# N3b3x/openballbot-rl

Measured on AMD Instinct MI355X. Metric: env-steps/sec at 4096 envs per GPU (flat terrain, random actions), higher is better.
Workload: dtype f64

## Files before the change

### openballbot-rl_amd/ballbot_gym/_native.py

```python
from __future__ import annotations

import ctypes as C
import os
from pathlib import Path

PKG = Path(__file__).resolve().parent
LIB_PATH = PKG / "_lib" / "libbb_mi355x.so"
SERIAL_LIB_PATH = PKG / "_lib" / "libbb_mi355x_serial.so"
SERIAL_FLAGS = ["-DBB_NO_TWIN_KIN", "-DBB_NO_TWIN_POS", "-DBB_NO_TWIN_BIAS", "-DBB_NO_MODEL_ONCE",
                "-DBB_NO_PRE_BATCH", "-DBB_NO_PRISM_WINDOW"]
CSRC = PKG.parent / "csrc"
INCLUDE = PKG.parent.parent / "include"

NQ, NV, NOBS, HF_N = 17, 15, 15, 293
DONE_TERMINATED, DONE_FAILURE, DONE_DIVERGED, DONE_OVERFLOW = 1, 2, 4, 8
NSTATS = 8
REWARD_DIRECTIONAL, REWARD_DISTANCE, REWARD_NONE = 0, 1, 2
DSBL_PASSIVE, DSBL_GRAVITY = 32, 64


class NativeLibraryError(RuntimeError):
    pass


class BBParams(C.Structure):
    _fields_ = [
        ("max_ep_steps", C.c_int),
        ("max_allowed_tilt", C.c_float),
        ("max_wheel_velocity", C.c_float),
        ("reward_scale", C.c_float),
        ("action_reg_coef", C.c_float),
        ("survival_bonus", C.c_float),
        ("target_dir", C.c_float * 2),
        ("reward_kind", C.c_int),
        ("goal", C.c_float * 2),
        ("goal_scale", C.c_float),
        ("n_terrains", C.c_int),
        ("seed", C.c_uint64),
        ("fp64", C.c_int),
        ("solver_maxiter", C.c_int),
        ("solver_tol", C.c_double),
        ("opt_timestep", C.c_double),
        ("opt_disableflags", C.c_int),
    ]


class PerlinCfg(C.Structure):
    _fields_ = [
        ("scale", C.c_double),
        ("octaves", C.c_int),
        ("persistence", C.c_float),
        ("lacunarity", C.c_float),
        ("amplitude", C.c_double),
    ]


class PPOMlpArgs(C.Structure):
    _fields_ = [(name, C.c_void_p) for name in ("params", "grad", "exp_avg", "exp_avg_sq")] + [
        ("n_params", C.c_int64),
        ("offsets", C.c_int32 * 21),
    ] + [(name, C.c_void_p) for name in ("obs", "actions", "old_logp", "advantages", "returns", "perm",
                                         "mb_counter", "row_counter", "log", "clip", "lr", "step", "coef")] + [
        ("B", C.c_int32),
# ... 232 lines not shown
```

### openballbot-rl_amd/csrc/bb_pid_rollout.hip

```cpp
#define BB_PID_TU
#ifndef BB_NO_PRE_BATCH
#define BB_NO_PRE_BATCH
#endif
#ifdef BB_PHASE_CLOCKS
#define bb_phase_cycles bb_phase_cycles_pid
#endif
#include "bb_kernels.hip"
```

### openballbot-rl_amd/csrc/bb_solve.h

```cpp
#pragma once

#include "bb_physics.h"

namespace bb {

#ifdef BB_SOLVE_STATS
static long g_ls_evals = 0;
static long g_ls_hist[16] = {0};
static long g_alpha1 = 0;
static long g_ls_snaps = 0;
static long g_ls_fallbacks = 0;
static int g_stage_iters[4] = {0, 0, 0, 0};
#endif

#if defined(BB_PHASE_CLOCKS) && defined(__HIP_DEVICE_COMPILE__)
extern __device__ unsigned long long bb_phase_cycles[100];
#define PH_DECL unsigned long long ph_t = clock64(), ph_acc[10] = {0, 0, 0, 0, 0, 0, 0, 0, 0, 0};
#define PH(k) { unsigned long long n_ = clock64(); ph_acc[k] += n_ - ph_t; ph_t = n_; }
#define PH_FLUSH(tm) if ((tm).tl == 0) { for (int k_ = 0; k_ < 8; k_++) atomicAdd(&bb_phase_cycles[k_], ph_acc[k_]); \
                                          atomicAdd(&bb_phase_cycles[32], ph_acc[8]); atomicAdd(&bb_phase_cycles[33], ph_acc[9]); }
#define PH_FLUSH_BODY(tm) if ((tm).tl == 0) { for (int k_ = 0; k_ < 10; k_++) atomicAdd(&bb_phase_cycles[80 + k_], ph_acc[k_]); }
#elif defined(BB_ISA_MARKS) && defined(__HIP_DEVICE_COMPILE__)
#define PH_DECL
#define PH(k) asm volatile("; PHASE_MARK " #k);
// ... 38 lines not shown
}

#ifdef __HIPCC__
__device__ __forceinline__ int team_shift_of(int L) { return (int(threadIdx.x) & 63) & ~(L - 1); }
#endif

BB_HD bool team_any(const Team& tm, bool b) {
#ifdef __HIP_DEVICE_COMPILE__
  const unsigned long long m = __ballot(b);
  const int sh = team_shift_of(tm.L);
  const unsigned long long mask = tm.L >= 64 ? ~0ull : ((1ull << tm.L) - 1);
  return ((m >> sh) & mask) != 0;
#else
  (void)tm;
  return b;
#endif
}

BB_HD void tri_unpack(int e, int& i, int& j) {
  int r = (int)((sqrtf(8.f * float(e) + 1.f) - 1.f) * 0.5f);
  while ((r + 1) * (r + 2) / 2 <= e) r++;
  while (r * (r + 1) / 2 > e) r--;
  i = r;
  j = e - r * (r + 1) / 2;
}

BB_HD void tri_unpack_count(int e, int& i, int& j) {
  int r = 0, s = 0;
#pragma unroll
  for (int k = 1; k < NV; k++) {
    const bool in = e >= k * (k + 1) / 2;
    r += in ? 1 : 0;
    s = in ? k * (k + 1) / 2 : s;
  }
  i = r;
  j = e - s;
}

template <typename T>
struct StageOut {
  T quat_b[4];
  T w_world[3];
  T v_com[3];
  T pb[3];
  int ng, nb, iters, overflow;
};

template <typename T>
struct TerrainRef {
  const float* hf;
  T size_z, hz;
};

template <typename T>
struct EnvWork {
  T q0[NQ], v0[NV], vs[NV], as[NV];
  T k1[NV];
  T qn[NQ], vn[NV], wn[NV];
  T qfs[NV];
  T vi[NV];
  StageOut<T> so;
  Mass<T> M;
  WheelCon<T> wc[3];
  T g[MAXG * NGF];
  T bc[MAXB_LDS * NBF];
  T* bspill;
#ifdef BB_PHASE_CLOCKS
  int dbg_nb;
#endif
  Poses<T> P;
  T H[NH];
  union U {
    struct {
      Kin<T> k;
      T Iw[3][6];
      T qi[NQ];
    } pre;
    struct {
      T cj[3][3][13];
      T wf[3][3];
      T hg[21];
    } hes;
  } u;
};

template <typename T>
BB_HD T* body_slot(T* bc, T* spill, int b) {
  return b < MAXB_LDS ? bc + b * NBF : spill + (b - MAXB_LDS) * NBF;
}

template <typename T>
BB_HD T mass_entry(const Mass<T>& M, int i, int j) {
  if (i < 3) return i == j ? M.mt : T(0);
  if (i < 6) {
    if (j < 3) return M.Mtr[3 * j + (i - 3)];
    const int a = i - 3, b = j - 3;
    return a == b ? M.Mrr[a] : M.Mrr[a + b + 2];
  }
  if (i < 9) {
    const int w = i - 6;
    if (j < 3) return M.Mth[w][j];
    if (j < 6) return M.Mrh[w][j - 3];
    return j == i ? M.Mhh[w] : T(0);
  }
  if (j < 9) return T(0);
  if (i < 12) return i == j ? M.mB : T(0);
  if (j < 12) return M.MBtr[3 * (j - 9) + (i - 12)];
  return i == j ? M.MBrr[i - 12] : T(0);
}

template <typename T>
BB_HD int mass_entry_off(int i, int j) {
  static_assert(sizeof(Mass<T>) == 53 * sizeof(T), "Mass<T> is 53 values of T, nothing else");
  constexpr int MT = offsetof(Mass<T>, mt) / sizeof(T), MTR = offsetof(Mass<T>, Mtr) / sizeof(T),
                MRR = offsetof(Mass<T>, Mrr) / sizeof(T), MTH = offsetof(Mass<T>, Mth) / sizeof(T),
                MRH = offsetof(Mass<T>, Mrh) / sizeof(T), MHH = offsetof(Mass<T>, Mhh) / sizeof(T),
                MB = offsetof(Mass<T>, mB) / sizeof(T), MBTR = offsetof(Mass<T>, MBtr) / sizeof(T),
                MBRR = offsetof(Mass<T>, MBrr) / sizeof(T);
  if (i < 3) return i == j ? MT : -1;
  if (i < 6) {
    if (j < 3) return MTR + 3 * j + (i - 3);
    const int a = i - 3, b = j - 3;
    return MRR + (a == b ? a : a + b + 2);
  }
  if (i < 9) {
    const int w = i - 6;
    if (j < 3) return MTH + 3 * w + j;
    if (j < 6) return MRH + 3 * w + (j - 3);
    return j == i ? MHH + w : -1;
  }
  if (j < 9) return -1;
  if (i < 12) return i == j ? MB : -1;
  if (j < 12) return MBTR + 3 * (j - 9) + (i - 12);
  return i == j ? MBRR + (i - 12) : -1;
}

BB_HD int wheel_pos(int i, int w) { return i < 6 ? i : (i == 6 + w ? 6 : (i >= 9 ? i - 2 : -1)); }
// ... 491 lines not shown
```

### openballbot-rl_amd/csrc/bb_step.h

```cpp
#pragma once

#include "bb_team16.h"

namespace bb {

#if defined(BB_ISA_MARKS) && defined(__HIP_DEVICE_COMPILE__)
#define BB_PRE(k) asm volatile("; PRE_MARK " #k);
#define BB_PRE_ARM(k, arm) asm volatile("; PRE_MARK " #k " " #arm);
#else
#define BB_PRE(k)
#define BB_PRE_ARM(k, arm)
#endif

struct EnvCfg {
  int max_ep_steps;
  float max_allowed_tilt;
  float max_wheel_velocity;
  float reward_scale;
  float action_reg_coef;
  float survival_bonus;
  float target[2];
  int reward_kind;
  float goal[2], goal_scale;
};
// ... 127 lines not shown
#endif
  } else {
    if (t16::body_candidates(m, k, tr.hf, tr.size_z, tr.hz, tm.tl, mo)) return -1;
  }
#else
  const int ng = tr.hf ? collide_ground(m, k, v, tr.hf, tr.size_z, st, &overflow) : 0;
#endif
#if defined(BB_PHASE_CLOCKS) && defined(__HIP_DEVICE_COMPILE__)
  if (tm.tl == 0) {
    const unsigned long long f_t2 = clock64();
    atomicAdd(&bb_phase_cycles[8], f_t1 - f_t0);
    atomicAdd(&bb_phase_cycles[9], f_t2 - f_t1);
    atomicAdd(&bb_phase_cycles[10], 1ull);
  }
#endif
  BB_PRE(7)
#pragma unroll
  for (int i = 0; i < 9; i++) { W.P.Rb[i] = k.Rb[i]; W.P.RB[i] = k.RB[i]; }
#pragma unroll
  for (int i = 0; i < 3; i++) { W.P.pb[i] = k.pb[i]; W.P.pB[i] = k.pB[i]; }
  if (so) {
    bool have_qb = false;
#if BB_TWIN_KIN && defined(__HIP_DEVICE_COMPILE__)
    have_qb = FUSE && tm.L == TWIN_L;
#endif
    if (!have_qb) {
      T qb[4] = {q[3], q[4], q[5], q[6]};
      qnormalize(qb);
      so->quat_b[0] = qb[0]; so->quat_b[1] = qb[1]; so->quat_b[2] = qb[2]; so->quat_b[3] = qb[3];
    }
    mv3(so->w_world, k.Rb, v + 3);
    T cl[3] = {M.mr[0] / M.mt, M.mr[1] / M.mt, M.mr[2] / M.mt}, cw[3], t[3];
    mv3(cw, k.Rb, cl);
    cross3(t, so->w_world, cw);
    so->v_com[0] = v[0] + t[0]; so->v_com[1] = v[1] + t[1]; so->v_com[2] = v[2] + t[2];
    so->pb[0] = q[0]; so->pb[1] = q[1]; so->pb[2] = q[2];
    so->ng = ng; so->overflow = overflow;
#ifdef __HIP_DEVICE_COMPILE__
    so->nb = nb;
#else
    so->nb = 0;
#endif
  }
  bool ok = true;
#pragma unroll
  for (int i = 0; i < NV; i++) ok = ok && isfinite(acc[i]);
  if (!ok) {
#pragma unroll
    for (int i = 0; i < NV; i++) acc[i] = 0;
  }
#ifdef __HIP_DEVICE_COMPILE__
  t16::mass_dense_team<FUSE && kPreBatchDense>(W, tm.tl);
  team_sync();
  if constexpr (!BODY) t16::ground_setup(m, W, ng, tm.tl);

#if defined(BB_PHASE_CLOCKS)
  const unsigned long long s_t0 = clock64();
#endif
#ifdef BB_EXP_DUP_SOLVE_FULL
  if constexpr (BODY) {
    T acc2[NV];
#pragma unroll
    for (int i = 0; i < NV; i++) acc2[i] = acc[i];
    (void)t16::solve16<BODY, FUSE>(m, W, ng, nb, acc2, tm.tl);
    asm volatile("" ::: "memory");
    team_sync();
  }
#endif
  BB_PRE(8)
  const int it = t16::solve16<BODY, FUSE>(m, W, ng, nb, acc, tm.tl);
  BB_PRE(9)
#if defined(BB_PHASE_CLOCKS)
  if (BODY && tm.tl == 0) {
    atomicAdd(&bb_phase_cycles[15], clock64() - s_t0);
    atomicAdd(&bb_phase_cycles[20], (unsigned long long)it);
  }
  if (tm.tl == 0) {
    atomicMax(&bb_phase_cycles[21], (unsigned long long)it);
    atomicAdd(&bb_phase_cycles[22 + (it / 2 < 9 ? it / 2 : 9)], 1ull);
  }
#endif
#else
  const int it = solve_team(m, W, W.qfs, ng, acc, tm);
#endif
  if (so) so->iters = it;
  return it;
}

template <typename T>
BB_HD bool vec_bad(const T* x, int n) {
  bool bad = false;
#pragma unroll
  for (int i = 0; i < n; i++) bad = bad || !(fabs(x[i]) <= T(1e10));
  return bad;
}

template <typename T>
BB_HD void rk_sums_batch(bool first, T b, const T* vi, const T* a, T* vs, T* as, T* k1) {
  T vl[NV], sv[NV], sa[NV];
#pragma unroll
  for (int i = 0; i < NV; i++) vl[i] = vi[i];
  if (first) {
    BB_ISSUE_FENCE();
#pragma unroll
    for (int i = 0; i < NV; i++) { sv[i] = b * vl[i]; sa[i] = b * a[i]; k1[i] = a[i]; }
  } else {
#pragma unroll
// ... 258 lines not shown
```

### openballbot-rl_amd/csrc/bb_team16.h

```cpp
#pragma once

#include <type_traits>
#include <utility>

#include "bb_bodycon.h"
#include "bb_solve.h"

namespace bb {

constexpr int LTR_SPARE = NV * (NV - 1) / 2, LTR_SLOTS = LTR_SPARE + 1;
BB_HD int ltr_slot(int tl, int k) {
  const int rw = tl < NV ? tl : 0;
  const int base = k < rw ? rw * (rw - 1) / 2 : LTR_SPARE - k;
  return base + k;
}

#ifdef __HIP_DEVICE_COMPILE__
namespace t16 {

constexpr int L = 16;

template <int CTRL>
__device__ __forceinline__ float dpp(float v) {
  return __int_as_float(__builtin_amdgcn_mov_dpp(__float_as_int(v), CTRL, 0xF, 0xF, true));
// ... 272 lines not shown
}

template <typename T>
__device__ __forceinline__ void body_load(const EnvWork<T>& W, int b, T (&o)[NBF]) {
  if (b < MAXB_LDS) {
    const T* p = W.bc + b * NBF;
#pragma unroll
    for (int i = 0; i < NBF; i++) o[i] = p[i];
  } else {
    const T* p = W.bspill + (b - MAXB_LDS) * NBF;
#pragma unroll
    for (int i = 0; i < NBF; i++) o[i] = p[i];
  }
}

template <bool BODY, typename T>
__device__ __forceinline__ void ls_terms(const ModelT<T>& m, const EnvWork<T>& W, int c, int ng, int nc, const T* a,
                                         const T* s, T (&c6)[6], T& D) {
#pragma unroll
  for (int r = 0; r < 6; r++) c6[r] = 0;
  D = 0;
  if (c >= nc) return;
  if (c < 3) {
    const WheelCon<T>& C = W.wc[c];
#pragma unroll
    for (int r = 0; r < 3; r++) { c6[r] = wheel_dot(C, c, r, a) - C.aref[r]; c6[3 + r] = wheel_dot(C, c, r, s); }
  } else if (c < 3 + ng) {
    T J[3][6], ar[3];
    ground_contact(m, W.g + (c - 3) * NGF, W.P.RB, W.vi, J, ar, D);
#pragma unroll
    for (int r = 0; r < 3; r++) { c6[r] = ground_dot(J, r, a) - ar[r]; c6[3 + r] = ground_dot(J, r, s); }
  } else if constexpr (BODY) {
    T bcv[NBF];
    body_load(W, c - 3 - ng, bcv);
    body_ls_terms(m, bcv, W.P, W.vi, a, s, c6, D);
  }
}

template <bool BODY, typename T>
__device__ __forceinline__ void ls_term(const ModelT<T>& m, const EnvWork<T>& W, int c, int ng, int nc, const T* a,
                                        const T* s, T kdw, LsTerm<T>& lt) {
  T c6[6], Dc;
  ls_terms<BODY>(m, W, c, ng, nc, a, s, c6, Dc);
  if (c >= nc) {
    lt.none();
    return;
  }
  const bool wheel = c < 3;
  const T D[3] = {wheel ? W.wc[c].D[0] : Dc, wheel ? W.wc[c].D[1] : Dc, wheel ? W.wc[c].D[2] : Dc};
  const T mu = wheel ? m.fr_wheel[0] : T(1), f1 = wheel ? m.fr_wheel[0] : T(1), f2 = wheel ? m.fr_wheel[1] : T(1);
  lt.prep(c6, c6 + 3, mu, f1, f2, D, D[0] * (wheel ? kdw : T(0.5)));
}

constexpr int GC_LDS = 13;
static_assert(GC_LDS * 18 <= MAXB_LDS * NBF, "ground Jacobians do not fit W.bc");

template <typename T>
__device__ __forceinline__ T* ground_ad(EnvWork<T>& W, int c) {
  static_assert(sizeof(Mass<T>) >= GC_LDS * 4 * sizeof(T), "ground aref/D do not fit the mass blocks");
  return reinterpret_cast<T*>(&W.M) + 4 * c;
}

template <typename T>
__device__ __forceinline__ void ground_setup(const ModelT<T>& m, EnvWork<T>& W, int ng, int tl) {
  const int c = tl - 3;
  if (c >= 0 && c < ng && c < GC_LDS) {
    T J[3][6], ar[3], D;
    ground_contact(m, W.g + c * NGF, W.P.RB, W.vi, J, ar, D);
    T* o = W.bc + c * 18;
#pragma unroll
    for (int r = 0; r < 3; r++)
#pragma unroll
      for (int i = 0; i < 6; i++) o[6 * r + i] = J[r][i];
    T* ad = ground_ad(W, c);
#pragma unroll
    for (int r = 0; r < 3; r++) ad[r] = ar[r];
    ad[3] = D;
  }
}

template <bool BODY, typename T>
__device__ __forceinline__ void ground_get(const ModelT<T>& m, EnvWork<T>& W, int c, T (&J)[3][6], T (&ar)[3], T& D) {
  if (!BODY && c < GC_LDS) {
    const T* o = W.bc + c * 18;
#pragma unroll
    for (int r = 0; r < 3; r++)
#pragma unroll
      for (int i = 0; i < 6; i++) J[r][i] = o[6 * r + i];
    const T* ad = ground_ad(W, c);
#pragma unroll
    for (int r = 0; r < 3; r++) ar[r] = ad[r];
    D = ad[3];
  } else {
    ground_contact(m, W.g + c * NGF, W.P.RB, W.vi, J, ar, D);
  }
}

#ifndef BB_NO_CARRY
constexpr bool kCarry = true;
#else
constexpr bool kCarry = false;
#endif

#ifndef BB_NO_LDS_BATCH_LS
constexpr bool kLdsBatchLs = true;
#else
constexpr bool kLdsBatchLs = false;
#endif
#ifndef BB_NO_LDS_BATCH_CP
constexpr bool kLdsBatchCp = true;
#else
constexpr bool kLdsBatchCp = false;
#endif
#ifndef BB_NO_LDS_BATCH_HESS
constexpr bool kLdsBatchHess = true;
#else
constexpr bool kLdsBatchHess = false;
#endif

#ifndef BB_NO_TAIL_UNIFORM
constexpr bool kTailUniform = true;
#else
constexpr bool kTailUniform = false;
#endif
#ifndef BB_NO_LS_SELECT
constexpr bool kLsSelect = true;
#else
constexpr bool kLsSelect = false;
#endif
#ifndef BB_NO_PREP_SELECT
constexpr bool kPrepSelect = true;
#else
constexpr bool kPrepSelect = false;
#endif

template <bool BODY, bool FUSE = false, typename T>
__device__ int solve16(const ModelT<T>& m, EnvWork<T>& W, int ng, int nb, T* a, int tl) {
  if constexpr (!BODY) nb = 0;
  const int ngc = 3 + ng;
  const int nc = ngc + nb;
  const bool rowl = tl < NV;
  const int row = rowl ? tl : NV - 1;
  const T muw = m.fr_wheel[0];
  T kdw;
#if BB_ONCE
  if constexpr (FUSE) kdw = once_of(m).kdw;
  else
#endif
    kdw = once_kdw(m);
  const T qfs_i = W.qfs[row];
  const int gcol = row - 9;
  static_assert(offsetof(typename EnvWork<T>::U, hes.hg) == offsetof(typename EnvWork<T>::U, hes.wf) + 9 * sizeof(T),
                "wheel f/C scratch needs wf and hg adjacent");
  T* const wCf = &W.u.hes.wf[0][0];
  const bool gsum = ng > 0;
#ifdef BB_HROW_REG
  T hM[NV];
#pragma unroll
  for (int k = 0; k < NV; k++) hM[k] = W.H[hidx(row, k)];
#define BB_HROW(k) hM[k]
#else
#define BB_HROW(k) W.H[hidx(row, k)]
#endif
  PH_DECL
  constexpr bool CARRY = kCarry && !BODY;
  constexpr bool UTAIL = FUSE && !BODY && kTailUniform;
  constexpr bool LSSEL = FUSE && !BODY && kLsSelect;
  constexpr bool PREPSEL = FUSE && !BODY && kPrepSelect;
  T jar0[3] = {0, 0, 0}, mq = 0;
  int it = 0;
  bool held = false;
  for (; it < m.maxiter; it++) {
    team_sync();
    PH_TOP
    int tlx = tl;
    asm volatile("" : "+v"(tlx));
    const bool fresh = !CARRY || it == 0;
    bool more = true;
    if constexpr (UTAIL) more = __ballot(nc > L) != 0;
    (void)more;
    T gg[6], Hg[21];
    auto cone_of = [&](bool wheel, int c, const T (&jar)[3], T Dc, T (&f)[3], T (&Cc)[6]) __attribute__((always_inline)) {
      const T D[3] = {wheel ? W.wc[c].D[0] : Dc, wheel ? W.wc[c].D[1] : Dc, wheel ? W.wc[c].D[2] : Dc};
      const T mu = wheel ? muw : T(1), f1 = wheel ? muw : T(1), f2 = wheel ? m.fr_wheel[1] : T(1);
      const T Dm = D[0] * (wheel ? kdw : T(0.5));
      cone_sel(jar, mu, f1, f2, D, Dm, f, Cc);
    };
    auto wheel_put = [&](int c, const T (&f)[3], const T (&Cc)[6]) __attribute__((always_inline)) {
      T* p = wCf + 9 * c;
#pragma unroll
      for (int r = 0; r < 6; r++) p[r] = Cc[r];
#pragma unroll
      for (int r = 0; r < 3; r++) p[6 + r] = f[r];
    };
    auto cj_of = [&](const T (&Cc)[6], const T (&Jg)[3][6], T (&w)[3][6]) __attribute__((always_inline)) {
#pragma unroll
      for (int i = 0; i < 6; i++) {
        w[0][i] = Cc[0] * Jg[0][i] + Cc[3] * Jg[1][i] + Cc[4] * Jg[2][i];
        w[1][i] = Cc[3] * Jg[0][i] + Cc[1] * Jg[1][i] + Cc[5] * Jg[2][i];
        w[2][i] = Cc[4] * Jg[0][i] + Cc[5] * Jg[1][i] + Cc[2] * Jg[2][i];
      }
    };
    auto partials = [&](const T (&Jg)[3][6], const T (&f)[3], const T (&w)[3][6]) __attribute__((always_inline)) {
#pragma unroll
      for (int i = 0; i < 6; i++) gg[i] -= Jg[0][i] * f[0] + Jg[1][i] * f[1] + Jg[2][i] * f[2];
#pragma unroll
      for (int i = 0; i < 6; i++)
#pragma unroll
        for (int j = 0; j <= i; j++) Hg[i * (i + 1) / 2 + j] += Jg[0][i] * w[0][j] + Jg[1][i] * w[1][j] + Jg[2][i] * w[2][j];
    };
    auto contact_pass = [&]() __attribute__((always_inline)) {
#pragma unroll
      for (int i = 0; i < 6; i++) gg[i] = 0;
#pragma unroll
      for (int i = 0; i < 21; i++) Hg[i] = 0;
      if constexpr (UTAIL) {
        if (tl < ngc) {
          const int c = tl;
          const bool wheel = c < 3;
          T jar[3] = {jar0[0], jar0[1], jar0[2]}, Dc = 0, Jg[3][6];
          if (!wheel) {
            T ar[3];
            ground_get<BODY>(m, W, c - 3, Jg, ar, Dc);
            if (fresh) {
#pragma unroll
              for (int r = 0; r < 3; r++) jar[r] = ground_dot(Jg, r, a) - ar[r];
            }
          } else if (fresh) {
            if constexpr (kLdsBatchCp) {
              wheel_jar3(W.wc[c], c, a, jar);
            } else {
#pragma unroll
              for (int r = 0; r < 3; r++) jar[r] = wheel_dot(W.wc[c], c, r, a) - W.wc[c].aref[r];
            }
          }
          if (fresh) {
#pragma unroll
            for (int r = 0; r < 3; r++) jar0[r] = jar[r];
          }
          T f[3], Cc[6];
          cone_of(wheel, c, jar, Dc, f, Cc);
          if (wheel) {
            wheel_put(c, f, Cc);
          } else {
            T w[3][6];
            cj_of(Cc, Jg, w);
            partials(Jg, f, w);
          }
        }
        if (more) {
          for (int c = tl + L; c < ngc; c += L) {
            T jar[3], Dc = 0, Jg[3][6], ar[3];
            ground_get<BODY>(m, W, c - 3, Jg, ar, Dc);
#pragma unroll
            for (int r = 0; r < 3; r++) jar[r] = ground_dot(Jg, r, a) - ar[r];
            T f[3], Cc[6], w[3][6];
            cone_of(false, c, jar, Dc, f, Cc);
            cj_of(Cc, Jg, w);
            partials(Jg, f, w);
          }
        }
      } else {
        for (int c = tl; c < ngc; c += L) {
          const bool wheel = c < 3;
          T jar[3] = {jar0[0], jar0[1], jar0[2]}, Dc = 0, Jg[3][6];
          if (!wheel) {
            T ar[3];
            ground_get<BODY>(m, W, c - 3, Jg, ar, Dc);
            if (fresh || c != tl) {
#pragma unroll
              for (int r = 0; r < 3; r++) jar[r] = ground_dot(Jg, r, a) - ar[r];
            }
          } else if (fresh) {
            if constexpr (FUSE && kLdsBatchCp) {
              wheel_jar3(W.wc[c], c, a, jar);
            } else {
#pragma unroll
              for (int r = 0; r < 3; r++) jar[r] = wheel_dot(W.wc[c], c, r, a) - W.wc[c].aref[r];
            }
          }
          if (fresh && c == tl) {
#pragma unroll
            for (int r = 0; r < 3; r++) jar0[r] = jar[r];
          }
          T f[3], Cc[6];
          cone_of(wheel, c, jar, Dc, f, Cc);
          if (wheel) {
            wheel_put(c, f, Cc);
          } else {
            T w[3][6];
            cj_of(Cc, Jg, w);
            partials(Jg, f, w);
          }
        }
      }
    };
#ifdef BB_EXP_DUP_CPASS
    {
      contact_pass();
      T z = 0;
      for (int i = 0; i < 6; i++) z += gg[i];
      for (int i = 0; i < 21; i++) z += Hg[i];
      asm volatile("" :: "v"(z) : "memory");
      team_sync();
    }
#endif
    contact_pass();
    T hb[NV], gb = 0;
#pragma unroll
    for (int i = 0; i < NV; i++) hb[i] = 0;
    if constexpr (BODY) {
#ifdef BB_EXP_DUP_FBODY
     for (int rep = 0; rep < 2; rep++) {
      if (rep == 1) { T z = 0; for (int i = 0; i < NV; i++) z += hb[i]; asm volatile("" :: "v"(z), "v"(gb) : "memory");
                      for (int i = 0; i < NV; i++) hb[i] = 0; gb = 0; }
#endif
      const bool r_ang = (row >= 3 && row < 6) || row >= 12, r_ball = row >= 9;
      const int r_h = (row >= 6 && row < 9) ? row - 6 : -2;
      const int r_e = row < 3 ? row : ((row >= 9 && row < 12) ? row - 9 : -1);
      T rc[3] = {0, 0, 0};
      if (r_ang) {
// ... 196 lines not shown
    };
#ifdef BB_EXP_DUP_HESS
    {
      T h2[NV];
#pragma unroll
      for (int k = 0; k < NV; k++) h2[k] = h[k] * T(0.5);
      wheel_blocks(h2);
      T acc = 0;
#pragma unroll
      for (int k = 0; k < NV; k++) acc += h2[k];
      asm volatile("" :: "v"(acc) : "memory");
    }
#endif
    wheel_blocks(h);
    if (gsum) {
#pragma unroll
      for (int ai = 0; ai < 6; ai++)
#pragma unroll
        for (int b = 0; b < 6; b++) {
          const T v = Hg[ai >= b ? ai * (ai + 1) / 2 + b : b * (b + 1) / 2 + ai];
          h[9 + b] += row == 9 + ai ? v : T(0);
        }
    }
    if constexpr (BODY) {
#pragma unroll
      for (int k = 0; k < NV; k++) h[k] += hb[k];
    }
    T hdi = 0;
#pragma unroll
    for (int k = 0; k < NV; k++) hdi = row == k ? h[k] : hdi;
    PH(3)
    T diag[NV], s[NV], sown;
#ifdef BB_EXP_DUP_CHOL
    {
      T h2[NV], d2[NV];
#pragma unroll
      for (int k = 0; k < NV; k++) h2[k] = h[k];
      chol_rows<FUSE>(h2, hdi, d2, tl);
      asm volatile("" :: "v"(d2[NV - 1]), "v"(h2[NV - 2]) : "memory");
    }
#endif
    chol_rows<FUSE>(h, hdi, diag, tl);
    PH(4)
#ifdef BB_EXP_DUP_TRSV
    {
      T s2[NV], so2;
      chol_solve_rows<FUSE, FUSE>(h, diag, gi, s2, so2, tl, &W.u.hes.cj[0][0][0]);
      asm volatile("" :: "v"(s2[0]), "v"(so2) : "memory");
      team_sync();
    }
#endif
    static_assert(sizeof(W.u.hes.cj) >= LTR_SLOTS * sizeof(T), "L's transpose and its spare slot do not fit cj");
    chol_solve_rows<FUSE, FUSE>(h, diag, gi, s, sown, tlx, &W.u.hes.cj[0][0][0]);
    T d0 = tsum(sown * gi);
    bool fin = true;
#pragma unroll
    for (int i = 0; i < NV; i++) fin = fin && isfinite(s[i]);
    if (!fin || !(d0 < 0)) {
      sown = rowl ? -gi / maxT(W.H[hidx(row, row)], T(1e-30)) : T(0);
      static_for<NV>([&](auto kc) {
        constexpr int k = decltype(kc)::value;
        s[k] = bcast<k>(sown);
      });
      d0 = tsum(sown * gi);
      if (!(d0 < 0)) break;
    }
    PH(5)
    T Ms = 0;
#pragma unroll
    for (int k = 0; k < NV; k++) Ms += BB_HROW(k) * s[k];
    const T sMs = tsum(sown * Ms), gs = tsum(sown * mq);
    LsTerm<T> lt;
    T x[3] = {0, 0, 0};
    if constexpr (PREPSEL) {
      const bool act = tl < ngc, wheel = tl < 3;
      T Dc[3] = {0, 0, 0};
      if (wheel) {
        const WheelCon<T>& C = W.wc[tl];
        if constexpr (kLdsBatchLs) {
          wheel_dot3(C, tl, s, x, C.D, Dc);
        } else {
#pragma unroll
          for (int r = 0; r < 3; r++) { x[r] = wheel_dot(C, tl, r, s); Dc[r] = C.D[r]; }
        }
      } else if (act) {
        T Jg[3][6], ar[3], D;
        ground_get<BODY>(m, W, tl - 3, Jg, ar, D);
#pragma unroll
        for (int r = 0; r < 3; r++) { x[r] = ground_dot(Jg, r, s); Dc[r] = D; }
      }
      const T one = act ? T(1) : T(0);
      const T mu = wheel ? muw : one, f1 = wheel ? muw : one, f2 = wheel ? m.fr_wheel[1] : one;
      const T j0[3] = {act ? jar0[0] : T(0), act ? jar0[1] : T(0), act ? jar0[2] : T(0)};
      lt.prep_sel(j0, x, mu, f1, f2, Dc, Dc[0] * (wheel ? kdw : T(0.5)));
    } else if (tl < ngc) {
      const bool wheel = tl < 3;
      T Dc[3];
      if (wheel) {
        const WheelCon<T>& C = W.wc[tl];
        if constexpr (FUSE && kLdsBatchLs) {
          wheel_dot3(C, tl, s, x, C.D, Dc);
        } else {
#pragma unroll
          for (int r = 0; r < 3; r++) { x[r] = wheel_dot(C, tl, r, s); Dc[r] = C.D[r]; }
        }
      } else {
        T Jg[3][6], ar[3], D;
        ground_get<BODY>(m, W, tl - 3, Jg, ar, D);
#pragma unroll
        for (int r = 0; r < 3; r++) { x[r] = ground_dot(Jg, r, s); Dc[r] = D; }
      }
      const T mu = wheel ? muw : T(1), f1 = wheel ? muw : T(1), f2 = wheel ? m.fr_wheel[1] : T(1);
      lt.prep(jar0, x, mu, f1, f2, Dc, Dc[0] * (wheel ? kdw : T(0.5)));
    } else {
      ls_term<BODY>(m, W, tl, ng, nc, a, s, kdw, lt);
    }
    LineSearch<T> lsr;
    bool ls_ok = false;
#ifdef BB_EXP_DUP_LS
    auto line_search = [&](LineSearch<T>& lsr, bool& ls_ok) {
      lsr.init(d0);
      ls_ok = false;
      for (int ls = 1; ls <= m.ls_maxiter; ls++) {
        const T alpha = lsr.alpha;
        T d1p = 0, d2p = 0, dmp = 0;
        lt.eval(alpha, d1p, d2p, dmp);
        for (int c = tl + L; c < nc; c += L) {
          LsTerm<T> lc;
          ls_term<BODY>(m, W, c, ng, nc, a, s, kdw, lc);
          lc.eval(alpha, d1p, d2p, dmp);
        }
        const T d1 = gs + alpha * sMs + tsum(d1p);
        const T d2 = sMs + tsum(d2p);
        const T dmag = fabs(gs) + fabs(alpha * sMs) + tsum(dmp);
        if (fabs(d1) <= m.ls_tol * fabs(d0) || fabs(d1) <= T(32) * eps_of<T>() * dmag) { ls_ok = true; break; }
        if (!(d1 == d1)) break;
        lsr.update(d1, d2);
        const bool up = lsr.alpha > lsr.prev;
        const T big = T(1e30);
        const T kv = tmin(lsr.crosses(lt.kink) ? (up ? lt.kink : -lt.kink) : big);
        const T ks = up ? kv : -kv;
        lsr.dx = kv < big ? fabs(ks - lsr.prev) : lsr.dx;
        lsr.alpha = kv < big ? ks : lsr.alpha;
      }
    };
    {
      LineSearch<T> l2;
      bool ok2;
      line_search(l2, ok2);
      asm volatile("" :: "v"(l2.alpha), "v"(int(ok2)) : "memory");
    }
    PH(8)
    line_search(lsr, ls_ok);
#else
    lsr.init(d0);
    PH(8)
    if constexpr (LSSEL) {
      bool done = false;
      for (int ls = 1; ls <= m.ls_maxiter && !done; ls++) {
        const T alpha = lsr.alpha;
        T p[3] = {0, 0, 0};
// ... 21 lines not shown
        for (int c = tl + L; c < nc; c += L) {
          LsTerm<T> lc;
          ls_term<BODY>(m, W, c, ng, nc, a, s, kdw, lc);
          lc.eval(alpha, d1p, d2p, dmp);
        }
      }
      const T d1 = gs + alpha * sMs + tsum(d1p);
      if (fabs(d1) <= m.ls_tol * fabs(d0)) { ls_ok = true; break; }
      const T dmag = fabs(gs) + fabs(alpha * sMs) + tsum(dmp);
      if (fabs(d1) <= T(32) * eps_of<T>() * dmag) { ls_ok = true; break; }
      if (!(d1 == d1)) break;
      const T d2 = sMs + tsum(d2p);
      lsr.update(d1, d2);
      const bool up = lsr.alpha > lsr.prev;
      const T big = T(1e30);
      const T kv = tmin(lsr.crosses(lt.kink) ? (up ? lt.kink : -lt.kink) : big);
      const T ks = up ? kv : -kv;
      lsr.dx = kv < big ? fabs(ks - lsr.prev) : lsr.dx;
      lsr.alpha = kv < big ? ks : lsr.alpha;
    }
    }
#endif
    if (!ls_ok) lsr.alpha = lsr.fallback();
    PH(9)
    const T alpha = lsr.alpha;
    if (!(alpha > 0)) break;
    T dc = lt.cost(alpha) - lt.cost(T(0));
    if (more) {
      for (int c = tl + L; c < nc; c += L) {
        LsTerm<T> lc;
        ls_term<BODY>(m, W, c, ng, nc, a, s, kdw, lc);
        dc += lc.cost(alpha) - lc.cost(T(0));
      }
    }
    const T dcost = alpha * (gs + T(0.5) * alpha * sMs) + tsum(dc);
    T sn = 0, an2 = 0;
#pragma unroll
    for (int i = 0; i < NV; i++) { a[i] += alpha * s[i]; sn += s[i] * s[i]; an2 += a[i] * a[i]; }
    if constexpr (CARRY) {
#pragma unroll
      for (int r = 0; r < 3; r++) jar0[r] += alpha * x[r];
      mq = rowl ? mq + alpha * Ms : T(0);
    }
    PH(6)
    if (alpha * alpha * sn <= T(1e-30) + m.step_rel2 * (1 + an2)) { it++; break; }
    if (-m.scale * dcost < m.tol) {
      const bool far = m.scale * m.scale * gn >= T(IMPR_GRAD * IMPR_GRAD) * m.tol * m.tol;
      if (!far || held) { it++; break; }
      held = true;
    }
  }
  PH(7)
#undef BB_HROW
  if constexpr (BODY) {
    PH_FLUSH_BODY((Team{L, tl}))
  } else {
    PH_FLUSH((Team{L, tl}))
  }
  return it;
}

template <typename T>
__device__ __forceinline__ int collide_team(const ModelT<T>& m, const Kin<T>& k, const T* v, const float* hf,
                                            T size_z, T* g, int* overflow, int tl,
                                            const ModelOnce<T>* mo = nullptr, T zbound = prism_no_bound<T>()) {
  const T r = m.ball_r;
  const T* c = k.c;
  const T sx = m.hf_sx, sy = m.hf_sy, zb = m.hf_bottom;
  const T zmin = c[2] - r;
  int cmin, cmax, rmin, rmax;
  if (!prism_window(m, c, size_z, zbound, cmin, cmax, rmin, rmax)) return 0;
  const int ncol = cmax - cmin + 1;
  const int np = 2 * ncol - 2;
  const int total = (rmax - rmin) * (np > 0 ? np : 0);
  T dx, dy;
  if (mo) { dx = mo->dx; dy = mo->dy; }
  else once_pitch(m, dx, dy);
  (void)v;
  const int team_shift = team_shift_of(L);
  int ng = 0;
  auto heights = [&](int P, float (&h)[3]) {
    if (P < total) {
      const int rr = rmin + P / np, p = P % np;
#pragma unroll
      for (int t = 0; t < 3; t++) {
        const int vt = p + t;
        h[t] = hf[(rr + (vt & 1)) * HF_N + cmin + (vt >> 1)];
      }
    }
  };
  float hnext[3] = {0.f, 0.f, 0.f};
  heights(tl, hnext);
  for (int base = 0; base < total; base += L) {
    const int P = base + tl;
    bool hit = false;
    T nn[3] = {0, 0, 1}, dist = 0;
    const float hcur[3] = {hnext[0], hnext[1], hnext[2]};
    heights(P + L, hnext);
    if (P < total) {
      const int rr = rmin + P / np, p = P % np;
      T V[3][3];
#pragma unroll
      for (int t = 0; t < 3; t++) {
        const int vt = p + t, cc = cmin + (vt >> 1), ri = rr + (vt & 1);
        V[t][0] = dx * cc - sx;
        V[t][1] = dy * ri - sy;
// ... 334 lines not shown
        const unsigned bits = unsigned(bal >> team_shift) & 0xFFFFu;
        if (cand_hit) cand[nc + __popc(bits & ((1u << tl) - 1u))] = code;
        nc += int(__popc(bits));
#if defined(BB_PHASE_CLOCKS) && defined(__HIP_DEVICE_COMPILE__)
        if (tl == 0) atomicAdd(&bb_phase_cycles[19], (unsigned long long)__popc(bits));
#endif
        if (nc > CAND_CAP - L) flush();
      }
#if defined(BB_PHASE_CLOCKS) && defined(__HIP_DEVICE_COMPILE__)
      if (tl == 0) {
        atomicAdd(&bb_phase_cycles[16], 1ull);
        atomicAdd(&bb_phase_cycles[17], (unsigned long long)total);
        atomicAdd(&bb_phase_cycles[18], (unsigned long long)((total + L - 1) / L));
      }
#endif
    }
    if (nc > 0) flush();
  }
  return nb;
}

template <bool BATCH = false, typename T>
__device__ __forceinline__ void mass_dense_team(EnvWork<T>& W, int tl) {
  if constexpr (BATCH) {
    constexpr int R = (NH + L - 1) / L;
    const T* Mp = reinterpret_cast<const T*>(&W.M);
    asm volatile("" : "+v"(tl));
    tl &= L - 1;
    int o[R];
    T x[R];
#pragma unroll
    for (int r = 0; r < R; r++) {
      const int e = tl + r * L;
      int i, j;
      tri_unpack_count(e < NH ? e : NH - 1, i, j);
      o[r] = mass_entry_off<T>(i, j);
      x[r] = Mp[o[r] < 0 ? 0 : o[r]];
    }
    BB_ISSUE_FENCE();
#pragma unroll
    for (int r = 0; r < R; r++) {
      const int e = tl + r * L;
      if (e < NH) W.H[e] = o[r] < 0 ? T(0) : x[r];
    }
  } else {
    for (int e = tl; e < NH; e += L) {
      int i, j;
      tri_unpack(e, i, j);
      W.H[e] = mass_entry(W.M, i, j);
    }
  }
}

}
#endif
}
```

Baseline: 14.42 million.

## Add square mass-row LDS copy, packed ground records, and fused triple reduction

Before the solve, each lane copies its row of the packed triangular Hessian into a square, bank-spread LDS layout so the per-iteration H·s row dot reads contiguous entries without index arithmetic or bank conflicts. Ground-contact Jacobians, aref and D are packed into one contiguous record per contact, placed in W.bc and the mass blocks. The three team reductions d0, sMs and gs are merged into one multi-value reduction, with Ms computed earlier. This reuses scratch regions, which is guarded by static_asserts, and adds a setup pass plus some register pressure.

```diff
diff --git a/openballbot-rl_amd/ballbot_gym/_native.py b/openballbot-rl_amd/ballbot_gym/_native.py
--- a/openballbot-rl_amd/ballbot_gym/_native.py
+++ b/openballbot-rl_amd/ballbot_gym/_native.py
@@ -8,7 +8,8 @@
 LIB_PATH = PKG / "_lib" / "libbb_mi355x.so"
 SERIAL_LIB_PATH = PKG / "_lib" / "libbb_mi355x_serial.so"
 SERIAL_FLAGS = ["-DBB_NO_TWIN_KIN", "-DBB_NO_TWIN_POS", "-DBB_NO_TWIN_BIAS", "-DBB_NO_MODEL_ONCE",
-                "-DBB_NO_PRE_BATCH", "-DBB_NO_PRISM_WINDOW"]
+                "-DBB_NO_PRE_BATCH", "-DBB_NO_PRISM_WINDOW", "-DBB_NO_HROW_SQUARE", "-DBB_NO_GROUND_RECORD",
+                "-DBB_NO_SUM3"]
 CSRC = PKG.parent / "csrc"
 INCLUDE = PKG.parent.parent / "include"
 
diff --git a/openballbot-rl_amd/csrc/bb_pid_rollout.hip b/openballbot-rl_amd/csrc/bb_pid_rollout.hip
--- a/openballbot-rl_amd/csrc/bb_pid_rollout.hip
+++ b/openballbot-rl_amd/csrc/bb_pid_rollout.hip
@@ -1,6 +1,15 @@
 #define BB_PID_TU
 #ifndef BB_NO_PRE_BATCH
 #define BB_NO_PRE_BATCH
+#endif
+#ifndef BB_NO_HROW_SQUARE
+#define BB_NO_HROW_SQUARE
+#endif
+#ifndef BB_NO_GROUND_RECORD
+#define BB_NO_GROUND_RECORD
+#endif
+#ifndef BB_NO_SUM3
+#define BB_NO_SUM3
 #endif
 #ifdef BB_PHASE_CLOCKS
 #define bb_phase_cycles bb_phase_cycles_pid
diff --git a/openballbot-rl_amd/csrc/bb_solve.h b/openballbot-rl_amd/csrc/bb_solve.h
--- a/openballbot-rl_amd/csrc/bb_solve.h
+++ b/openballbot-rl_amd/csrc/bb_solve.h
@@ -114,6 +114,30 @@
   T size_z, hz;
 };
 
+#ifndef BB_NO_HROW_SQUARE
+constexpr bool kHrowSquare = true;
+#else
+constexpr bool kHrowSquare = false;
+#endif
+#ifndef BB_NO_GROUND_RECORD
+constexpr bool kGroundRecord = true;
+#else
+constexpr bool kGroundRecord = false;
+#endif
+constexpr int GC_LDS = 13;
+constexpr int HS = NV;
+constexpr int HSQ_H_ROWS = 12, HSQ_G_PAD = 2, HSQ_G_STRIDE = HS + 2;
+constexpr int HX = kHrowSquare ? HSQ_H_ROWS * HS - NH : 0;
+static_assert(HS % 2 == 1 && HSQ_H_ROWS * HS >= NH, "square rows: odd stride, the packed triangle inside them");
+static_assert(HSQ_G_PAD + (NV - 1 - HSQ_H_ROWS) * HSQ_G_STRIDE + HS <= GC_LDS * NGF,
+              "the last rows of the square copy do not fit the stored contacts' head of W.g");
+constexpr int GREC = 22, GREC_AREF = 18, GREC_D = 21;
+constexpr int GREC_BC = MAXB_LDS * NBF / GREC;
+static_assert(GREC_BC <= GC_LDS && (GC_LDS - GREC_BC) * GREC <= int(sizeof(Mass<double>) / sizeof(double)),
+              "ground records do not fit W.bc and the mass blocks");
+static_assert(GC_LDS * 18 <= MAXB_LDS * NBF && int(sizeof(Mass<double>) / sizeof(double)) >= GC_LDS * 4,
+              "ground Jacobians do not fit W.bc, or aref/D the mass blocks (-DBB_NO_GROUND_RECORD)");
+
 template <typename T>
 struct EnvWork {
   T q0[NQ], v0[NV], vs[NV], as[NV];
@@ -131,7 +155,7 @@
   int dbg_nb;
 #endif
   Poses<T> P;
-  T H[NH];
+  T H[NH + HX];
   union U {
     struct {
       Kin<T> k;
@@ -145,6 +169,31 @@
     } hes;
   } u;
 };
+
+template <typename T>
+BB_HD constexpr int hsq_row_off(int i) {
+  return i < HSQ_H_ROWS ? int(offsetof(EnvWork<T>, H) / sizeof(T)) + i * HS
+                        : int(offsetof(EnvWork<T>, g) / sizeof(T)) + HSQ_G_PAD + (i - HSQ_H_ROWS) * HSQ_G_STRIDE;
+}
+template <typename T>
+BB_HD constexpr int grec_off(int c) {
+  return c < GREC_BC ? int(offsetof(EnvWork<T>, bc) / sizeof(T)) + c * GREC
+                     : int(offsetof(EnvWork<T>, M) / sizeof(T)) + (c - GREC_BC) * GREC;
+}
+template <typename T>
+BB_HD T* ws_at(EnvWork<T>& W, int off) { return reinterpret_cast<T*>(&W) + off; }
+template <typename T>
+BB_HD const T* ws_at(const EnvWork<T>& W, int off) { return reinterpret_cast<const T*>(&W) + off; }
+constexpr bool hsq_rows_spread() {
+  bool seen[16] = {};
+  for (int i = 0; i < NV; i++) {
+    const int r = hsq_row_off<double>(i) % 16;
+    if (seen[r]) return false;
+    seen[r] = true;
+  }
+  return true;
+}
+static_assert(!kHrowSquare || hsq_rows_spread(), "two rows of the square copy share a bank pair");
 
 template <typename T>
 BB_HD T* body_slot(T* bc, T* spill, int b) {
diff --git a/openballbot-rl_amd/csrc/bb_step.h b/openballbot-rl_amd/csrc/bb_step.h
--- a/openballbot-rl_amd/csrc/bb_step.h
+++ b/openballbot-rl_amd/csrc/bb_step.h
@@ -203,7 +203,8 @@
 #ifdef __HIP_DEVICE_COMPILE__
   t16::mass_dense_team<FUSE && kPreBatchDense>(W, tm.tl);
   team_sync();
-  if constexpr (!BODY) t16::ground_setup(m, W, ng, tm.tl);
+  if constexpr (!BODY) t16::ground_setup<FUSE>(m, W, ng, tm.tl);
+  if constexpr (!BODY && FUSE && kHrowSquare) t16::mass_rows_team(W, tm.tl);
 
 #if defined(BB_PHASE_CLOCKS)
   const unsigned long long s_t0 = clock64();
diff --git a/openballbot-rl_amd/csrc/bb_team16.h b/openballbot-rl_amd/csrc/bb_team16.h
--- a/openballbot-rl_amd/csrc/bb_team16.h
+++ b/openballbot-rl_amd/csrc/bb_team16.h
@@ -348,42 +348,49 @@
   lt.prep(c6, c6 + 3, mu, f1, f2, D, D[0] * (wheel ? kdw : T(0.5)));
 }
 
-constexpr int GC_LDS = 13;
-static_assert(GC_LDS * 18 <= MAXB_LDS * NBF, "ground Jacobians do not fit W.bc");
 
 template <typename T>
 __device__ __forceinline__ T* ground_ad(EnvWork<T>& W, int c) {
-  static_assert(sizeof(Mass<T>) >= GC_LDS * 4 * sizeof(T), "ground aref/D do not fit the mass blocks");
   return reinterpret_cast<T*>(&W.M) + 4 * c;
 }
-
-template <typename T>
+template <bool REC, typename T>
+__device__ __forceinline__ T* ground_j(EnvWork<T>& W, int c) {
+  return REC ? ws_at(W, grec_off<T>(c)) : W.bc + c * 18;
+}
+template <bool REC, typename T>
+__device__ __forceinline__ T* ground_aref(EnvWork<T>& W, int c, T* j) {
+  return REC ? j + GREC_AREF : ground_ad(W, c);
+}
+
+template <bool FUSE = false, typename T>
 __device__ __forceinline__ void ground_setup(const ModelT<T>& m, EnvWork<T>& W, int ng, int tl) {
+  constexpr bool REC = FUSE && kGroundRecord;
   const int c = tl - 3;
   if (c >= 0 && c < ng && c < GC_LDS) {
     T J[3][6], ar[3], D;
     ground_contact(m, W.g + c * NGF, W.P.RB, W.vi, J, ar, D);
-    T* o = W.bc + c * 18;
+    T* o = ground_j<REC>(W, c);
 #pragma unroll
     for (int r = 0; r < 3; r++)
 #pragma unroll
       for (int i = 0; i < 6; i++) o[6 * r + i] = J[r][i];
-    T* ad = ground_ad(W, c);
+    T* ad = ground_aref<REC>(W, c, o);
 #pragma unroll
     for (int r = 0; r < 3; r++) ad[r] = ar[r];
     ad[3] = D;
   }
 }
 
-template <bool BODY, typename T>
+template <bool BODY, bool FUSE = false, typename T>
 __device__ __forceinline__ void ground_get(const ModelT<T>& m, EnvWork<T>& W, int c, T (&J)[3][6], T (&ar)[3], T& D) {
+  constexpr bool REC = FUSE && kGroundRecord;
   if (!BODY && c < GC_LDS) {
-    const T* o = W.bc + c * 18;
+    const T* o = ground_j<REC>(W, c);
 #pragma unroll
     for (int r = 0; r < 3; r++)
 #pragma unroll
       for (int i = 0; i < 6; i++) J[r][i] = o[6 * r + i];
-    const T* ad = ground_ad(W, c);
+    const T* ad = ground_aref<REC>(W, c, const_cast<T*>(o));
 #pragma unroll
     for (int r = 0; r < 3; r++) ar[r] = ad[r];
     D = ad[3];
@@ -428,6 +435,12 @@
 constexpr bool kPrepSelect = true;
 #else
 constexpr bool kPrepSelect = false;
+#endif
+
+#ifndef BB_NO_SUM3
+constexpr bool kSum3 = true;
+#else
+constexpr bool kSum3 = false;
 #endif
 
 template <bool BODY, bool FUSE = false, typename T>
@@ -450,13 +463,16 @@
                 "wheel f/C scratch needs wf and hg adjacent");
   T* const wCf = &W.u.hes.wf[0][0];
   const bool gsum = ng > 0;
+  constexpr bool SQ = kHrowSquare && FUSE && !BODY;
+  const T* const hrow = SQ ? ws_at(W, hsq_row_off<T>(row)) : W.H;
+#define BB_HROW_LDS(k) (SQ ? hrow[k] : W.H[hidx(row, k)])
 #ifdef BB_HROW_REG
   T hM[NV];
 #pragma unroll
-  for (int k = 0; k < NV; k++) hM[k] = W.H[hidx(row, k)];
+  for (int k = 0; k < NV; k++) hM[k] = BB_HROW_LDS(k);
 #define BB_HROW(k) hM[k]
 #else
-#define BB_HROW(k) W.H[hidx(row, k)]
+#define BB_HROW(k) BB_HROW_LDS(k)
 #endif
   PH_DECL
   constexpr bool CARRY = kCarry && !BODY;
@@ -517,7 +533,7 @@
           T jar[3] = {jar0[0], jar0[1], jar0[2]}, Dc = 0, Jg[3][6];
           if (!wheel) {
             T ar[3];
-            ground_get<BODY>(m, W, c - 3, Jg, ar, Dc);
+            ground_get<BODY, FUSE>(m, W, c - 3, Jg, ar, Dc);
             if (fresh) {
 #pragma unroll
               for (int r = 0; r < 3; r++) jar[r] = ground_dot(Jg, r, a) - ar[r];
@@ -547,7 +563,7 @@
         if (more) {
           for (int c = tl + L; c < ngc; c += L) {
             T jar[3], Dc = 0, Jg[3][6], ar[3];
-            ground_get<BODY>(m, W, c - 3, Jg, ar, Dc);
+            ground_get<BODY, FUSE>(m, W, c - 3, Jg, ar, Dc);
 #pragma unroll
             for (int r = 0; r < 3; r++) jar[r] = ground_dot(Jg, r, a) - ar[r];
             T f[3], Cc[6], w[3][6];
@@ -562,7 +578,7 @@
           T jar[3] = {jar0[0], jar0[1], jar0[2]}, Dc = 0, Jg[3][6];
           if (!wheel) {
             T ar[3];
-            ground_get<BODY>(m, W, c - 3, Jg, ar, Dc);
+            ground_get<BODY, FUSE>(m, W, c - 3, Jg, ar, Dc);
             if (fresh || c != tl) {
 #pragma unroll
               for (int r = 0; r < 3; r++) jar[r] = ground_dot(Jg, r, a) - ar[r];
@@ -865,24 +881,43 @@
 #endif
     static_assert(sizeof(W.u.hes.cj) >= LTR_SLOTS * sizeof(T), "L's transpose and its spare slot do not fit cj");
     chol_solve_rows<FUSE, FUSE>(h, diag, gi, s, sown, tlx, &W.u.hes.cj[0][0][0]);
-    T d0 = tsum(sown * gi);
+    constexpr bool SUM3 = FUSE && kSum3;
+    T d0, Ms = 0, sMs = 0, gs = 0;
+    if constexpr (SUM3) {
+#pragma unroll
+      for (int k = 0; k < NV; k++) Ms += BB_HROW(k) * s[k];
+      T p3[3] = {sown * gi, sown * Ms, sown * mq};
+      tsum_n(p3);
+      d0 = p3[0]; sMs = p3[1]; gs = p3[2];
+    } else {
+      d0 = tsum(sown * gi);
+    }
     bool fin = true;
 #pragma unroll
     for (int i = 0; i < NV; i++) fin = fin && isfinite(s[i]);
     if (!fin || !(d0 < 0)) {
-      sown = rowl ? -gi / maxT(W.H[hidx(row, row)], T(1e-30)) : T(0);
+      sown = rowl ? -gi / maxT(SQ ? hrow[row] : W.H[hidx(row, row)], T(1e-30)) : T(0);
       static_for<NV>([&](auto kc) {
         constexpr int k = decltype(kc)::value;
         s[k] = bcast<k>(sown);
       });
       d0 = tsum(sown * gi);
       if (!(d0 < 0)) break;
+      if constexpr (SUM3) {
+        Ms = 0;
+#pragma unroll
+        for (int k = 0; k < NV; k++) Ms += BB_HROW(k) * s[k];
+        sMs = tsum(sown * Ms);
+        gs = tsum(sown * mq);
+      }
     }
     PH(5)
-    T Ms = 0;
-#pragma unroll
-    for (int k = 0; k < NV; k++) Ms += BB_HROW(k) * s[k];
-    const T sMs = tsum(sown * Ms), gs = tsum(sown * mq);
+    if constexpr (!SUM3) {
+#pragma unroll
+      for (int k = 0; k < NV; k++) Ms += BB_HROW(k) * s[k];
+      sMs = tsum(sown * Ms);
+      gs = tsum(sown * mq);
+    }
     LsTerm<T> lt;
     T x[3] = {0, 0, 0};
     if constexpr (PREPSEL) {
@@ -898,7 +933,7 @@
         }
       } else if (act) {
         T Jg[3][6], ar[3], D;
-        ground_get<BODY>(m, W, tl - 3, Jg, ar, D);
+        ground_get<BODY, FUSE>(m, W, tl - 3, Jg, ar, D);
 #pragma unroll
         for (int r = 0; r < 3; r++) { x[r] = ground_dot(Jg, r, s); Dc[r] = D; }
       }
@@ -919,7 +954,7 @@
         }
       } else {
         T Jg[3][6], ar[3], D;
-        ground_get<BODY>(m, W, tl - 3, Jg, ar, D);
+        ground_get<BODY, FUSE>(m, W, tl - 3, Jg, ar, D);
 #pragma unroll
         for (int r = 0; r < 3; r++) { x[r] = ground_dot(Jg, r, s); Dc[r] = D; }
       }
@@ -1047,6 +1082,7 @@
   }
   PH(7)
 #undef BB_HROW
+#undef BB_HROW_LDS
   if constexpr (BODY) {
     PH_FLUSH_BODY((Team{L, tl}))
   } else {
@@ -1487,6 +1523,18 @@
   }
 }
 
-}
-#endif
-}
+template <typename T>
+__device__ __forceinline__ void mass_rows_team(EnvWork<T>& W, int tl) {
+  const int row = tl < NV ? tl : NV - 1;
+  T x[NV];
+#pragma unroll
+  for (int k = 0; k < NV; k++) x[k] = W.H[hidx(row, k)];
+  BB_ISSUE_FENCE();
+  T* o = ws_at(W, hsq_row_off<T>(row));
+#pragma unroll
+  for (int k = 0; k < NV; k++) o[k] = x[k];
+}
+
+}
+#endif
+}
```

After: 14.71 million (median of 6 runs). +2.0%, better.
